# bigpon/QPNet

Hardware: AMD Instinct MI355X
Metric: train steps/sec (batch-1 chunk-steps of RF+20000 samples, aggregate over GPUs) (higher is better)
Workload: dtype f32; 1 GPU; config[1]: paper-size SI-QPNet (C=64,S=256,4F+4A) training step, forward+CE+backward+Adam on one chunk of 20900 samples (RF 946 + batch_length 19954), batch 1 per GPU; global_batch=1, parallelism=dp1 (utterance-sharded chunks, one flat-gradient all-reduce per step), backend=none, world_size=1, aux_1x1=frame rate (hoisted: K = 128 + one 4-deep step)

## Files before the change

qpnet_amd/csrc/train_bwd.hip:

```cpp
#include "train_common.h"
#include "train_post.h"
#include "qpn_handle.h"
#include <string.h>
#include <stdlib.h>
#include <math.h>

template <int MT>
__global__ __launch_bounds__(512) void k_post_bwd(TrainParams p, TrainBwd bw) {
    constexpr int TM = 16 * MT;
    extern __shared__ float sm[];
    const int S = p.S, Q = p.Q, LC = p.LC;
    const int ldp = tr_lda(Q > S ? Q : S), ldr = tr_lda(S);
    float* P = sm; float* R = sm + TM * ldp;
    const int b = blockIdx.y, t0 = blockIdx.x * TM;
    const int tid = threadIdx.x, lane = tid & 63, wave = tid >> 6;
    const int NTS = S / 16;
    const int npairs = (NTS + 1) / 2;
    const int np0 = wave < npairs ? wave : 0;
    const int pnt[2] = {2 * np0, (2 * np0 + 1 < NTS) ? 2 * np0 + 1 : 2 * np0};
    float my[2][MT][4], ms[2][MT][4];
    auto mask_load = [&](const float* src, float (&m)[2][MT][4]) {
#pragma unroll
        for (int j = 0; j < 2; ++j)
#pragma unroll
// ... 414 lines not shown
        }
        if constexpr (HOIST) {
            if (lane < 16) {
                float* dp = bw.DPA + cpoff + 16 * wave + lane;
                atomicAdd(dp, dacc[0]); atomicAdd(dp + C, dacc[1]); atomicAdd(dp + 2 * C, dacc[2]); atomicAdd(dp + 3 * C, dacc[3]);
                float* ep = bw.EB + (size_t)(l * TR_EB_SLOTS + (blockIdx.x & (TR_EB_SLOTS - 1))) * 2 * C + 16 * wave + lane;
                atomicAdd(ep, eacc[0]); atomicAdd(ep + C, eacc[1]);
            }
            if (tid < 16 && n0 + tid < N1) GWl[n0 + tid] = (Gp[tid] + Gp[16 + tid]) + (Gp[32 + tid] + Gp[48 + tid]);
        }
        store_rows(t + 1 < t_last ? t + 1 : t_last, sm + ((ti + 1) & 1) * 4 * 16 * ldx);
#pragma unroll
        for (int i = 0; i < 4; ++i) tprow[i] = tpnext[i];
        if constexpr (HOIST) {
#pragma unroll
            for (int i = 0; i < 4; ++i) { cwj[i] = nwj[i]; cpa[i] = npa[i]; }
            cpoff = npoff;
        }
    }
}

struct Wg2 {
    const float* A; const float* A2; size_t A_lstride; int lda, M;
    int rowsA;
    int bmode; const float* B1; const float* B2; size_t B_lstride; int ldb, N, Nvalid;
    int rowsB;
    const float* hup; const int* tap; int C, Ap;
    const int* xc;
    int nb, nlayers;
    float* slab; int gstage;
    int row0A[TR_MAXL], row0B[TR_MAXL], R[TR_MAXL];
    int goff[TR_MAXL], gbias[TR_MAXL], tap_off[TR_MAXL], dil[TR_MAXL];
    int ldc, ncol_groups;
};

struct Wg2L {
    const float* A; const float* A2; const float* B1; const float* B2; const float* hup; const int* tap;
    int lda, ldb, M, Ng, Nvalid, rowsA, rowsB, row0A, row0B, C, Ap, dil, nb, ncol0, rend;
    unsigned uR;
};

template <int NB>
__device__ __forceinline__ void wg_taps(const Wg2L& q, int rs, int (&tp)[NB], bool b_act, int b_row0, int b_rstep) {
#pragma unroll
    for (int k = 0; k < NB; ++k) {
        const int r = b_row0 + k * b_rstep, rr = rs + r;
        int v = 0;
        if (b_act && r < 32 && rr < q.rend) {
            const unsigned b = q.nb > 1 ? (unsigned)rr / q.uR : 0u; const int i = rr - (int)(b * q.uR);
            const int nloc = q.row0B + i;
            v = q.tap ? q.tap[(size_t)b * q.rowsB + nloc] : nloc - q.dil;
        }
        tp[k] = v;
    }
}

template <int BMODE, int NA, int NB>
__device__ __forceinline__ void wg_fetch(const Wg2L& q, int rs, float4 (&ra)[NA], float4 (&ra2)[NA], float4 (&rb)[NB], float4 (&rb2)[NB], const int (&tpv)[NB],
                                         bool a_act, int a_row0, int a_rstep, int a_col, bool b_act, int b_row0, int b_rstep, int b_col) {
#pragma unroll
    for (int k = 0; k < NA; ++k) {
        const int r = a_row0 + k * a_rstep, rr = rs + r;
        float4 v = make_float4(0.f, 0.f, 0.f, 0.f), v2 = v;
        if (a_act && r < 32 && rr < q.rend && a_col < q.M) {
            const unsigned b = q.nb > 1 ? (unsigned)rr / q.uR : 0u; const int i = rr - (int)(b * q.uR);
            const size_t o = ((size_t)b * q.rowsA + q.row0A + i) * q.lda + a_col;
// ... 155 lines not shown
    __shared__ float hcol[64];
    __shared__ float red[4];
    const int U = p.U, Ap = p.Ap, A = p.A;
    const int64_t q0 = (int64_t)p.F * U - p.N1;
    const int f = (int)(q0 / U) + fx;
    float dsum = 0.f;
    for (int a0 = 0; a0 < A; a0 += 64) {
        __syncthreads();
        if (tid < 64) hcol[tid] = (a0 + tid < A && f < p.F) ? p.h[((size_t)b * A + a0 + tid) * p.F + f] : 0.f;
        __syncthreads();
        for (int j = tid; j < U; j += nthr) {
            const int64_t n = (int64_t)f * U + j - q0;
            if (n < 0 || n >= p.N1 || f >= p.F) continue;
            const float* row = p.DHUP + ((size_t)b * p.N1 + n) * Ap + a0;
            float acc = 0.f;
            const int na = A - a0 < 64 ? A - a0 : 64;
            const int nq = na >> 2;
            float4 v[16];
#pragma unroll
            for (int q = 0; q < 16; ++q) v[q] = *(const float4*)(row + 4 * (q < nq ? q : 0));
#pragma unroll
            for (int q = 0; q < 16; ++q)
                if (q < nq) { acc += v[q].x * hcol[4 * q] + v[q].y * hcol[4 * q + 1] + v[q].z * hcol[4 * q + 2] + v[q].w * hcol[4 * q + 3]; dsum += (v[q].x + v[q].y) + (v[q].z + v[q].w); }
            for (int a = 4 * nq; a < na; ++a) { const float v1 = row[a]; acc += v1 * hcol[a]; dsum += v1; }
            atomicAdd(&p.gflat[p.up_w + j], acc * p.gscale);
        }
    }
    for (int s = 32; s >= 1; s >>= 1) dsum += __shfl_xor(dsum, s);
    if ((tid & 63) == 0) red[tid >> 6] = dsum;
    __syncthreads();
    if (tid == 0) { float a = 0.f; for (int k = 0; k < nthr / 64; ++k) a += red[k]; atomicAdd(&p.gflat[p.up_b], a * p.gscale); }
}

template <int BMODE, int MPW, int NT, bool TWO_A>
__device__ __forceinline__ void wgrad3_body(const Wg2& w, const int nch, const int ch, const int y, const int zg) {
    extern __shared__ float sm[];
    constexpr int RS = 32, Mp = 64 * MPW, Np = 16 * NT;
    constexpr int ldA = ((Mp + 15) / 32) * 32 + 16, ldB = ((Np + 15) / 32) * 32 + 16;
    constexpr int A4 = Mp / 4, ARS = 256 / A4, NA = RS / ARS;
    constexpr int B4 = Np / 4, BRS = 256 / B4, NB = (RS + BRS - 1) / BRS;
    static_assert(256 % A4 == 0 && RS % ARS == 0, "A staging must tile the stage's rows exactly");
    constexpr int BUF = RS * (ldA + ldB);
    float* As = sm; float* Bs = sm + RS * ldA;
    const int tid = threadIdx.x, lane = tid & 63, wave = tid >> 6;
    const int Rl = w.R[y];
    const int64_t total = (int64_t)Rl * w.nb;
    const int64_t per = ((total + nch - 1) / nch + RS - 1) / RS * RS;
    const int rbeg = (int)(per * ch), rend = (int)(per * ch + per < total ? per * ch + per : total);
    const float* A = w.A + (size_t)y * w.A_lstride;
    const float* A2 = TWO_A ? w.A2 + (size_t)y * w.A_lstride : nullptr;
    const float* B1 = BMODE == 4 ? nullptr : w.B1 + (size_t)y * w.B_lstride;
    const float* B2 = w.B2 ? w.B2 + (size_t)y * w.B_lstride : nullptr;
    const int* tap = BMODE == 3 ? w.tap + w.tap_off[y] : nullptr;
    const int row0A = w.row0A[y], row0B = w.row0B[y], ncol0 = zg * Np;
    const unsigned uR = (unsigned)(Rl > 0 ? Rl : 1);
    const bool multi = w.nb > 1;
    const int gbias = zg == 0 ? w.gbias[y] : -1, goff = w.goff[y];
    const int a_col = (tid % A4) * 4, a_row0 = tid / A4;
    const int b_col = (tid % B4) * 4, b_row0 = tid / B4;
    const int n = ncol0 + b_col;
    const bool b_act = tid < BRS * B4;
    const bool b_pad = n >= w.Nvalid;
    const float* bbase; int bstride; bool use_tap = false;
    if (BMODE == 3) {
        if (n < w.C) { bbase = B1 + n; bstride = w.C; }
        else if (n < 2 * w.C) { bbase = B1 + (n - w.C); bstride = w.C; use_tap = true; }
        else { bbase = w.hup + (b_pad ? 0 : n - 2 * w.C); bstride = w.Ap; }
    } else if (BMODE == 4) { bbase = nullptr; bstride = 0; }
    else { bbase = B1 + n; bstride = w.ldb; }
    const ptrdiff_t b2off = (BMODE == 2) ? (B2 - B1) : 0;

    f32x4 acc[MPW][NT];
#pragma unroll
    for (int a = 0; a < MPW; ++a)
#pragma unroll
        for (int b = 0; b < NT; ++b) acc[a][b] = (f32x4){0, 0, 0, 0};
    float4 cs4 = make_float4(0.f, 0.f, 0.f, 0.f);
    float4 ra[NA], ra2[NA], rb[NB], rb2[NB];
    int tpv[NB];
    int rbi[NB];
    unsigned okA = 0, okB = 0;

    const unsigned a_voff = (unsigned)a_row0 * (unsigned)w.lda + (unsigned)a_col, a_kstep = (unsigned)ARS * (unsigned)w.lda;
    const unsigned b_voff = (unsigned)b_row0 * (unsigned)w.ldb + (unsigned)n, b_kstep = (unsigned)BRS * (unsigned)w.ldb;

    auto rowsplit = [&](int rr, int& b, int& i) { if (multi) { b = (int)((unsigned)rr / uR); i = rr - b * (int)uR; } else { b = 0; i = rr; } };
    auto stage_fast = [&](int rs, int& b0, int& i0) {
        rowsplit(rs, b0, i0);
        return rs + RS <= rend && i0 + RS <= (int)uR;
    };
    auto taps = [&](int rs) {
        int b0, i0;
        if (stage_fast(rs, b0, i0)) {
            const int* tst = tap + ((size_t)b0 * w.rowsB + row0B + i0);
#pragma unroll
            for (int k = 0; k < NB; ++k) { const int r = b_row0 + k * BRS; tpv[k] = tst[r < RS ? r : b_row0]; }
            return;
        }
#pragma unroll
        for (int k = 0; k < NB; ++k) {
            const int r = b_row0 + k * BRS;
            int rr = rs + r; rr = rr < rend ? rr : rend - 1;
            int b, i; rowsplit(rr, b, i);
            const int nloc = row0B + i;
            tpv[k] = tap[(size_t)b * w.rowsB + nloc];
        }
    };
    auto fetch = [&](int rs) {
        const float* pa[NA]; const float* pb[NB]; const int* pi[NB];
        int b0, i0;
        if (stage_fast(rs, b0, i0)) {
            const float* Ast = A + ((size_t)b0 * w.rowsA + row0A + i0) * w.lda;
#pragma unroll
            for (int k = 0; k < NA; ++k) pa[k] = Ast + (k * a_kstep + a_voff);
            okA = ~0u;
            const size_t brow = (size_t)b0 * w.rowsB + row0B + i0;
            const float* bsrc = BMODE == 3 ? bbase + (size_t)b0 * w.rowsB * bstride : B1 + brow * w.ldb;
#pragma unroll
            for (int k = 0; k < NB; ++k) {
                const int r = b_row0 + k * BRS;
                if (BMODE == 4) pi[k] = w.xc + brow + (r < RS ? r : b_row0);
                else if (BMODE == 3) {
                    const unsigned row = use_tap ? (unsigned)tpv[k] : (unsigned)(row0B + i0 + (r < RS ? r : b_row0));
                    pb[k] = bsrc + __umul24(row, (unsigned)bstride);
                } else pb[k] = bsrc + ((r < RS ? k * b_kstep : 0u) + b_voff);
            }
            okB = b_pad ? 0u : ~0u;
        } else {
            okA = 0; okB = 0;
#pragma unroll
            for (int k = 0; k < NA; ++k) {
                const int r = a_row0 + k * ARS;
                int rr = rs + r; const bool ok = rr < rend; rr = ok ? rr : rend - 1;
                int b, i; rowsplit(rr, b, i);
                pa[k] = A + (((size_t)b * w.rowsA + row0A + i) * w.lda + a_col);
                okA |= ok ? 1u << k : 0u;
            }
#pragma unroll
            for (int k = 0; k < NB; ++k) {
                const int r = b_row0 + k * BRS;
                int rr = rs + r; const bool ok = r < RS && rr < rend && !b_pad; rr = rr < rend ? rr : rend - 1;
                int b, i; rowsplit(rr, b, i);
                const size_t row = (size_t)b * w.rowsB + ((BMODE == 3 && use_tap) ? tpv[k] : row0B + i);
                if (BMODE == 4) pi[k] = w.xc + row; else pb[k] = bbase + row * bstride;
                okB |= ok ? 1u << k : 0u;
            }
        }
#pragma unroll
        for (int k = 0; k < NA; ++k) {
            ra[k] = *(const float4*)pa[k];
            if (TWO_A) ra2[k] = *(const float4*)(pa[k] + (A2 - A));
        }
        if (b_act) {
#pragma unroll
            for (int k = 0; k < NB; ++k) {
                if (BMODE == 4) rbi[k] = *pi[k];
                else {
                    rb[k] = *(const float4*)pb[k];
                    if (BMODE == 2) rb2[k] = *(const float4*)(pb[k] + b2off);
                }
            }
        }
    };
    if (rbeg < rend) {
        if (BMODE == 3) taps(rbeg);
        fetch(rbeg);
        if (BMODE == 3 && rbeg + RS < rend) taps(rbeg + RS);
    }
    const int g = lane >> 4, cl = lane & 15;
    auto to_lds = [&](int buf) {
        float* Ab = As + buf * BUF; float* Bb = Bs + buf * BUF;
#pragma unroll
        for (int k = 0; k < NA; ++k) {
            float4 v = ra[k];
            if (TWO_A) { v.x += ra2[k].x; v.y += ra2[k].y; v.z += ra2[k].z; v.w += ra2[k].w; }
            { const bool ok = (okA >> k) & 1u; v.x = ok ? v.x : 0.f; v.y = ok ? v.y : 0.f; v.z = ok ? v.z : 0.f; v.w = ok ? v.w : 0.f; }
            cs4.x += v.x; cs4.y += v.y; cs4.z += v.z; cs4.w += v.w;
            *(float4*)(Ab + (size_t)(a_row0 + k * ARS) * ldA + a_col) = v;
        }
        if (b_act) {
#pragma unroll
            for (int k = 0; k < NB; ++k) {
                const int r = b_row0 + k * BRS;
                if (r < RS) {
                    float4 v;
                    if (BMODE == 4) { const int dlt = rbi[k] - n; v = make_float4(dlt == 0 ? 1.f : 0.f, dlt == 1 ? 1.f : 0.f, dlt == 2 ? 1.f : 0.f, dlt == 3 ? 1.f : 0.f); }
                    else v = rb[k];
                    if (BMODE == 1) { v.x = fmaxf(v.x, 0.f); v.y = fmaxf(v.y, 0.f); v.z = fmaxf(v.z, 0.f); v.w = fmaxf(v.w, 0.f); }
                    else if (BMODE == 2) { v.x *= rb2[k].x; v.y *= rb2[k].y; v.z *= rb2[k].z; v.w *= rb2[k].w; }
                    { const bool ok = (okB >> k) & 1u; v.x = ok ? v.x : 0.f; v.y = ok ? v.y : 0.f; v.z = ok ? v.z : 0.f; v.w = ok ? v.w : 0.f; }
                    *(float4*)(Bb + (size_t)r * ldB + b_col) = v;
                }
            }
        }
    };
    auto ksteps = [&](int buf, int k0, int k1) {
        const float* Ab = As + buf * BUF; const float* Bb = Bs + buf * BUF;
#pragma unroll
        for (int ks = k0; ks < k1; ++ks) {
            float bfr[NT];
#pragma unroll
            for (int nt = 0; nt < NT; ++nt) bfr[nt] = Bb[(4 * ks + g) * ldB + 16 * nt + cl];
#pragma unroll
            for (int mi = 0; mi < MPW; ++mi) {
                const float a = Ab[(4 * ks + g) * ldA + 16 * (wave + 4 * mi) + cl];
#pragma unroll
                for (int nt = 0; nt < NT; ++nt) acc[mi][nt] = __builtin_amdgcn_mfma_f32_16x16x4f32(a, bfr[nt], acc[mi][nt], 0, 0, 0);
            }
        }
    };
    for (int rs = rbeg; rs < rend; rs += RS) {
        to_lds(0);
        __syncthreads();
        if (rs + RS < rend) {
            fetch(rs + RS);
            if (BMODE == 3 && rs + 2 * RS < rend) taps(rs + 2 * RS);
        }
        ksteps(0, 0, RS / 4);
        __syncthreads();
    }
    float* out = w.slab + (size_t)ch * w.gstage;
#pragma unroll
    for (int mi = 0; mi < MPW; ++mi) {
        const int mt = wave + 4 * mi;
#pragma unroll
        for (int nt = 0; nt < NT; ++nt) {
#pragma unroll
            for (int i = 0; i < 4; ++i) {
                const int m = 16 * mt + 4 * (lane >> 4) + i, nn = 16 * nt + (lane & 15);
                out[goff + (size_t)m * w.ldc + ncol0 + nn] = acc[mi][nt][i];
            }
        }
    }
    if (gbias >= 0) {
        *(float4*)(sm + (size_t)a_row0 * Mp + a_col) = cs4;
        __syncthreads();
        if (tid < Mp) { float s = 0.f; for (int r = 0; r < ARS; ++r) s += sm[r * Mp + tid]; out[gbias + tid] = s; }
    }
}
template <int BMODE, int MPW, int NT, bool TWO_A, int MINW = 1>
__global__ __launch_bounds__(256, MINW) void k_wgrad3(Wg2 w, int nch) {
    wgrad3_body<BMODE, MPW, NT, TWO_A>(w, nch, blockIdx.x, blockIdx.y, blockIdx.z);
}

#ifndef QPN_WGRAD_MINW
#define QPN_WGRAD_MINW 2
#endif
template <int BMODE, int MPW, int NT, bool TWO_A>
static void launch_wgrad3_k(const Wg2& w, int nch, size_t lds, hipStream_t stream) {
    constexpr int MINW = (MPW == 4 && NT == 4 && !TWO_A) ? QPN_WGRAD_MINW : 1;
    if (lds > 64 * 1024) (void)hipFuncSetAttribute((const void*)k_wgrad3<BMODE, MPW, NT, TWO_A, MINW>, hipFuncAttributeMaxDynamicSharedMemorySize, (int)lds);
    hipLaunchKernelGGL((k_wgrad3<BMODE, MPW, NT, TWO_A, MINW>), dim3(nch, w.nlayers, w.ncol_groups), dim3(256), lds, stream, w, nch);
}
template <int BMODE, int MPW, int NT>
static bool wgrad3_fits(const Wg2& w) {
    const int Ng = w.N / w.ncol_groups;
    if (w.bmode != BMODE) return false;
    if (w.rowsB >= (1 << 24) || (int64_t)w.rowsB * (w.C > w.ldb ? w.C : w.ldb) >= (1ll << 32)) return false;
    if (w.M != 64 * MPW || Ng != 16 * NT || w.N % w.ncol_groups || (w.Nvalid != w.N && (w.ncol_groups != 1 || w.Nvalid % 4))) return false;
    if (BMODE == 3 && (w.ldb != w.C || w.ncol_groups != 1 || (w.C % 4) || (w.Ap % 4) || !w.tap)) return false;
    if (BMODE == 3) for (int l = 0; l < w.nlayers; ++l) if (w.tap_off[l] < 0) return false;
    return true;
}
template <int MPW, int NT> static constexpr size_t wgrad3_lds() { return (size_t)32 * (tr_ldt(64 * MPW) + tr_ldt(16 * NT)) * sizeof(float); }
template <int BMODE, int MPW, int NT>
static bool launch_wgrad3(const Wg2& w, int nch, hipStream_t stream) {
    if (!wgrad3_fits<BMODE, MPW, NT>(w)) return false;
    const size_t lds = wgrad3_lds<MPW, NT>();
    if (w.A2) launch_wgrad3_k<BMODE, MPW, NT, true>(w, nch, lds, stream);
    else launch_wgrad3_k<BMODE, MPW, NT, false>(w, nch, lds, stream);
    return true;
}
static bool wgrad3_any(const Wg2& w, int nch, bool generic, hipStream_t stream) {
    if (w.bmode == 4) return launch_wgrad3<4, 1, 8>(w, nch, stream) || launch_wgrad3<4, 1, 4>(w, nch, stream);
    if (generic) return false;
    switch (w.bmode) {
    case 3: return launch_wgrad3<3, 2, 11>(w, nch, stream) || launch_wgrad3<3, 2, 8>(w, nch, stream) || launch_wgrad3<3, 1, 7>(w, nch, stream);
    case 0: return launch_wgrad3<0, 1, 4>(w, nch, stream) || launch_wgrad3<0, 4, 4>(w, nch, stream);
    case 1: return launch_wgrad3<1, 4, 4>(w, nch, stream);
    default: return false;
    }
}

static int wgrad_col_groups(int M, int N) {
    const int nt_max = M <= 64 ? 4 : M <= 128 ? 12 : 8;
    for (int g = 1; g <= N / 16; ++g)
        if (N % g == 0 && (N / g) % 4 == 0 && (N / g + 15) / 16 <= nt_max) return g;
    return 1;
}

static bool wgrad2_any(const Wg2& w, int nch, bool generic, hipStream_t stream) {
    if (w.M > 256 && w.bmode != 4) {
        bool ok = true;
        for (int m0 = 0; m0 < w.M && ok; m0 += 256) {
            Wg2 sub = w;
            sub.A = w.A + m0; if (w.A2) sub.A2 = w.A2 + m0;
            sub.M = w.M - m0 < 256 ? w.M - m0 : 256;
            for (int l = 0; l < w.nlayers; ++l) { sub.goff[l] = w.goff[l] + m0 * w.ldc; if (w.gbias[l] >= 0) sub.gbias[l] = w.gbias[l] + m0; }
            sub.ncol_groups = wgrad_col_groups(sub.M, sub.N);
            ok = wgrad2_any(sub, nch, generic, stream);
        }
        return ok;
    }
    if (wgrad3_any(w, nch, generic, stream)) return true;
    switch (w.bmode) {
    case 4: return false;
    case 1: return wgrad2_mode<1>(w, nch, stream);
    case 2: return wgrad2_mode<2>(w, nch, stream);
    case 3: return wgrad2_mode<3>(w, nch, stream);
    default: return wgrad2_mode<0>(w, nch, stream);
    }
}

__global__ void k_reduce_grad_s(const float* __restrict__ slab, const int* __restrict__ gdst, const int* __restrict__ gdst_list, const int* __restrict__ gzero, int n_gzero,
                                int nch, int gstage, int64_t n, float* __restrict__ g, float scale, int append_scale, int s0, int s1, int skip0, int skip1, int tail,
                                const int* __restrict__ status, int flag_again) {
    int64_t i = (int64_t)blockIdx.x * blockDim.x + threadIdx.x + s0;
    if (flag_again && append_scale && i == s0) g[n + 1] = (status && *status) ? 1.f : 0.f;
    if (i < s1) {
        if (i >= skip0 && i < skip1) return;
        const int k0 = gdst[i], k1 = gdst[i + 1];
        if (k0 == k1) return;
        float a = 0.f;
        const float* sp = slab + i;
        int c = 0;
        for (; c + 8 <= nch; c += 8) {
            float v[8];
#pragma unroll
            for (int k = 0; k < 8; ++k) v[k] = sp[(size_t)(c + k) * gstage];
            a += ((v[0] + v[1]) + (v[2] + v[3])) + ((v[4] + v[5]) + (v[6] + v[7]));
        }
        for (; c < nch; ++c) a += sp[(size_t)c * gstage];
        a *= scale;
        for (int k = k0; k < k1; ++k) g[gdst_list[k]] = a;
        return;
    }
    if (!tail) return;
// ... 279 lines not shown
    hipLaunchKernelGGL((k_post_fb_w<MTW>), dim3((p.BL + 16 * MTW - 1) / (16 * MTW), p.B), dim3(512), ldsw, stream, p, bw, 1);
}

int qpn_launch_bwd(const TrainParams& p, const TrainBwd& bw, const TrainKnobs& k, const AuxGeom& ag, const StackQ* sq, hipStream_t stream, bool post_done) {
    const int C = p.C, S = p.S, Q = p.Q, L = p.L, B = p.B, N1 = p.N1, BL = p.BL;
    const TrainSlabs& sl = *bw.sl;
    const bool off32 = N1 < (1 << 24) && (int64_t)N1 * (p.LC > 2 * C ? p.LC : 2 * C) < (1ll << 32);
    const bool persist = C == 64 && (p.Ktp == 176 || p.hoist) && p.Ap <= 64 && off32 && k.persist_bwd;
    const bool stack_q = persist && k.stack_q_bwd && sq && sq->flags && p.qctl && qpn_stack_bwd_fits(p);
    const bool wr_summed = stack_q;
    const size_t nDX = (size_t)B * N1 * C;
    const size_t lds_post = (size_t)16 * (tr_lda(Q > S ? Q : S) + tr_lda(S)) * sizeof(float);
    const size_t lds_layer = (size_t)16 * (4 * tr_lda(C) + tr_lda(2 * C)) * sizeof(float);
    if (lds_post > 160 * 1024 || lds_layer > 160 * 1024) { qpn_set_error("backward tiles do not fit LDS"); return QPN_EINVAL; }
    hipStream_t side = bw.side; hipEvent_t ev_fork = bw.ev_fork, ev_join = bw.ev_join;
    const bool overlap = side && !qpn_prof_serial() && !k.serial;
    const bool post_wide = S == 256 && Q == 256 && C == 64 && (p.LC == 256 || p.LC == 512) && k.post_wide;
    const bool zero_in_post = post_wide && k.zero_in_post;
    if (post_done) { }
    else if (!zero_in_post) qpn_launch_zero_dx(p, bw, stream);
    if (post_done) { }
    else if (post_wide) {
        constexpr int MTW = 5;
        const size_t ldsw = (size_t)16 * MTW * tr_lda(256) * sizeof(float);
        QPN_HIP(hipFuncSetAttribute((const void*)k_post_bwd_w<MTW>, hipFuncAttributeMaxDynamicSharedMemorySize, (int)ldsw));
        hipLaunchKernelGGL((k_post_bwd_w<MTW>), dim3((BL + 16 * MTW - 1) / (16 * MTW), B), dim3(512), ldsw, stream, p, bw, zero_in_post ? 1 : 0);
    } else {
        if (lds_post > 48 * 1024) (void)hipFuncSetAttribute((const void*)k_post_bwd<1>, hipFuncAttributeMaxDynamicSharedMemorySize, (int)lds_post);
        hipLaunchKernelGGL((k_post_bwd<1>), dim3((BL + 15) / 16, B), dim3(512), lds_post, stream, p, bw);
    }
    qpn_prof_mark(PG_POST_BWD, stream);
    const int nch = bw.nch;
    int nch_side_ = nch;
    const bool gen = k.wgrad_generic;
    Wg2 wbase; memset(&wbase, 0, sizeof(wbase));
    wbase.slab = bw.slab; wbase.gstage = bw.gstage; wbase.nb = B; wbase.C = C; wbase.Ap = p.Ap; wbase.hup = p.HUP; wbase.tap = p.TAP; wbase.ncol_groups = 1;
    bool ok = true;
    auto launch_skip_post = [&](hipStream_t st) {
        Wg2 w = wbase;
        {
            w.nlayers = L;
            w.A = bw.DS0; w.A2 = nullptr; w.A_lstride = 0; w.lda = S; w.M = S; w.rowsA = BL;
            w.bmode = 0; w.B1 = p.TH; w.B2 = nullptr; w.B_lstride = nDX; w.ldb = C; w.N = C; w.Nvalid = C; w.rowsB = N1; w.ldc = C;
            w.ncol_groups = wgrad_col_groups(w.M, w.N);
            for (int l = 0; l < L; ++l) { w.row0A[l] = 0; w.row0B[l] = N1 - BL; w.R[l] = BL; w.goff[l] = sl.g_ws[l]; w.gbias[l] = l == 0 ? sl.g_bs : -1; w.tap_off[l] = -1; }
            ok = ok && wgrad2_any(w, nch_side_, gen, st);
            qpn_prof_mark(PG_WGRAD_SKIP, st);
        }
        {
            w.nlayers = 1; w.A_lstride = w.B_lstride = 0; w.B2 = nullptr; w.bmode = 1; w.rowsA = w.rowsB = BL;
            w.row0A[0] = w.row0B[0] = 0; w.R[0] = BL; w.tap_off[0] = -1;
            w.ncol_groups = S % 64 == 0 ? S / 64 : 1;
            w.A = bw.dlogits; w.lda = Q; w.M = Q; w.B1 = p.Y0; w.ldb = S; w.N = S; w.Nvalid = S; w.ldc = S; w.goff[0] = sl.g_p2; w.gbias[0] = sl.g_bp2;
            if (Q == S && k.post_pair) {
                w.nlayers = 2;
                w.A_lstride = (size_t)(bw.DY0 - bw.dlogits); w.B_lstride = (size_t)(p.S0 - p.Y0);
                w.row0A[1] = w.row0B[1] = 0; w.R[1] = BL; w.tap_off[1] = -1; w.goff[1] = sl.g_p1; w.gbias[1] = sl.g_bp1;
                ok = ok && wgrad2_any(w, nch_side_, gen, st);
            } else {
                ok = ok && wgrad2_any(w, nch_side_, gen, st);
                w.A = bw.DY0; w.lda = S; w.M = S; w.B1 = p.S0; w.goff[0] = sl.g_p1; w.gbias[0] = sl.g_bp1;
                ok = ok && wgrad2_any(w, nch_side_, gen, st);
            }
            qpn_prof_mark(PG_WGRAD_POST, st);
        }
    };
    auto build_w1 = [&]() {
        Wg2 w = wbase;
// ... 117 lines not shown
```

qpnet_amd/csrc/train_common.h:

```cpp
#pragma once
#include "qpn_common.h"

typedef float f32x4 __attribute__((ext_vector_type(4)));

#define TR_MAXL QPN_MAX_LAYERS

__host__ __device__ static inline int tr_lda(int K) { return ((K + 29) / 32) * 32 + 2; }
__host__ __device__ static inline int tr_ldt(int N) { return ((N + 15) / 32) * 32 + 16; }

struct TrLayer {
    int adaptive, dilation;
    int s_in, s_out;
    int tap_off;
    int w1_f4, wr_f4;
    int w1t_f4, wrt_f4;
    int bias1, biasr;
};

struct TrainParams {
    int C, S, Q, A, Ap, L, U;
    int B, T, F, Td, BL, N1, N0, maxd;
    int Kt, Ktp;
    int LC;
    const float* flat;
// ... 48 lines not shown
    float* slab;
    const int* gdst; const int* gdst_list;
    const int* gzero; int n_gzero;
    int nch, gstage;
    int64_t n_params;
    const struct TrainSlabs* sl;
    float gscale;
    int append_scale;
    const int* status;
    hipStream_t side; hipEvent_t ev_fork, ev_join, ev_mid;
    hipEvent_t ev_early; int* early_recorded;
};


struct AuxGeom { int auxS[TR_MAXL], auxT[TR_MAXL], bias1[TR_MAXL], s_out[TR_MAXL]; };
struct AuxArgs {
    const float* flat; const float* h; float* PA; float* bp; const float* DPA; const float* EB; const float* GW; float* gflat;
    float gscale; int C, A, L, B, F, U, N1, nfr, ffirst; int64_t up_w, up_b;
    AuxGeom g;
};
static inline AuxArgs tr_aux_args(const TrainParams& p, const TrainBwd* bw, const AuxGeom& ag) {
    AuxArgs a; a.flat = p.flat; a.h = p.h; a.PA = p.PA; a.bp = p.bp; a.DPA = bw ? bw->DPA : nullptr; a.EB = bw ? bw->EB : nullptr; a.GW = bw ? bw->GW : nullptr;
    a.gflat = bw ? bw->gflat : nullptr; a.gscale = bw ? bw->gscale : 1.f;
    a.C = p.C; a.A = p.A; a.L = p.L; a.B = p.B; a.F = p.F; a.U = p.U; a.N1 = p.N1; a.nfr = p.nfr; a.ffirst = p.ffirst; a.up_w = p.up_w; a.up_b = p.up_b; a.g = ag;
    return a;
}
struct TrainKnobs {
    bool serial;
    bool stack_q_fwd, stack_q_bwd;
    int stack_wgs, stack_wgs_bwd;
    bool persist_fwd, persist_bwd;
    bool wgrad_generic;
    int wgrad_chunks, wgrad_chunks_side;
    bool post_fuse;
    bool up_side, reduce_early, wr_side;
    bool post_pair, zero_in_post, post_wide;
    bool xcd_swizzle;
    bool ce_separate;
    bool event_fence;
    bool aux_hoist;
    bool test_stack_gives_up;
};
void qpn_train_knobs_parse(TrainKnobs& k);

#define TR_QHEAD_STRIDE 1056
#define TR_QHDR_WORDS 17920
struct StackQ {
    unsigned* flags;
    unsigned* head;
    unsigned* stats;
    unsigned* abort;
    const int4* tab;
    unsigned epoch;
    unsigned epoch_pub;
    unsigned spin_limit;
    int total, nq;
};

__host__ __device__ __forceinline__ int tr_pa_off(const TrainParams& p, int l, int b, int n0) {
    const int q = p.F * p.U - p.N1 + n0;
    return ((l * p.B + b) * (p.nfr + 1) + (q / p.U - p.ffirst)) * 2 * p.C;
}

__device__ __forceinline__ void tr_queue_entry_fwd(const TrainParams& p, int pos, int4& a, int4& b) {
    const bool valid = pos < p.qtotal;
    const int ps = valid ? pos : 0;
// ... 259 lines not shown
```

qpnet_amd/csrc/train_host.hip:

```cpp
#include "train_common.h"
#include "qpn_handle.h"
#include <algorithm>
#include <string.h>

int qpn_launch_fwd(const TrainParams& p, const TrainKnobs& k, const AuxGeom& ag, const StackQ* sq, hipStream_t stream, const TrainBwd* fuse_post_bwd);
void qpn_stack_fill(TrainParams& p);
int qpn_launch_ce(const float* logits, const int64_t* tgt, int64_t tgt_stride, int B, int BL, int Q, float* dlogits, double* loss, int* status, bool loss_cleared, hipStream_t stream);
int qpn_launch_bwd(const TrainParams& p, const TrainBwd& bw, const TrainKnobs& k, const AuxGeom& ag, const StackQ* sq, hipStream_t stream, bool post_done);
int qpn_launch_fwd_gemm(const TrainParams& p, const TrainGemm& w, hipStream_t stream);
int qpn_launch_bwd_gemm(const TrainParams& p, const TrainBwd& bw, const TrainGemm& w, hipStream_t stream);
int qpn_launch_adam(float* w, const float* g, float* m, float* v, int64_t n, int step, float lr, float b1, float b2, float eps, float wd, const float* den, int* status,
                    int* h_status, double* h_loss, const double* d_loss, hipStream_t stream);
int qpn_launch_adam_clip(float* w, const float* g, float* m, float* v, int64_t n, int step, float lr, float b1, float b2, float eps, float wd, const float* den, int* status,
                         int* h_status, double* h_loss, const double* d_loss, float max_norm, double* part, double* d_norm, double* h_norm, hipStream_t stream);

#define LOSS_SLOT 72

struct TrainState {
    std::vector<int> h_wmap;
    std::vector<int> h_bstart, h_blist;
    std::vector<int> h_gsrc;
    int* d_wmap; float* d_wp; int* d_bstart; int* d_blist; float* d_bp; int n_bias;
    int* d_gdst; int* d_gdst_list; int* d_gzero; int n_gzero;
    bool hoist;
// ... 10 lines not shown
    double* h_loss_pinned; hipEvent_t ev_loss[2]; bool loss_pending[2]; int loss_newest;
    double* d_gnorm; bool gnorm_last;
    bool gnorm_slot[2];
    double gnorm_collected; bool gnorm_collected_valid;
    bool fwd_valid;
    bool loss_clear;
    bool use_gemm;
    int* d_ctmap; float* d_ct;
    std::vector<int> h_gmap; int* d_gmap; float* d_gwp;
    TrainGemm gm;
    int64_t generation;
    hipStream_t side; hipEvent_t ev_fork, ev_join, ev_mid;
    hipEvent_t ev_early; int early_recorded; int64_t early_first;
    int64_t bwd_generation;
    const float* post_bwd_dlogits;
    bool post_bwd_done;
    bool stack_disabled;
    unsigned* d_sq; size_t sq_pos_cap, sq_per_dir;
    StackQ sqf, sqb;
};

static int env_int(const char* name, int dflt) { const char* e = getenv(name); return (e && *e) ? atoi(e) : dflt; }
void qpn_train_knobs_parse(TrainKnobs& k) {
    k.serial = env_int("QPN_TRAIN_SERIAL", 0) != 0;
    k.stack_q_fwd = env_int("QPN_STACK_QUEUE", 1) != 0;
    k.stack_q_bwd = k.stack_q_fwd && env_int("QPN_STACK_QUEUE_BWD", 1) != 0;
    k.stack_wgs = env_int("QPN_STACK_WGS", 0); if (k.stack_wgs < 0 || k.stack_wgs > 4096) k.stack_wgs = 0;
    k.stack_wgs_bwd = env_int("QPN_STACK_WGS_BWD", 0); if (k.stack_wgs_bwd < 0 || k.stack_wgs_bwd > 4096) k.stack_wgs_bwd = 0;
    k.persist_fwd = env_int("QPN_LAYER_PERSIST", 1) != 0;
    k.persist_bwd = env_int("QPN_LAYER_BWD_PERSIST", 1) != 0;
    k.wgrad_generic = getenv("QPN_WGRAD_GENERIC") != nullptr;
    k.wgrad_chunks = env_int("QPN_WGRAD_CHUNKS", 0); if (k.wgrad_chunks < 1 || k.wgrad_chunks > 512) k.wgrad_chunks = 0;
    k.wgrad_chunks_side = env_int("QPN_WGRAD_CHUNKS_SIDE", 0); if (k.wgrad_chunks_side < 1 || k.wgrad_chunks_side > 512) k.wgrad_chunks_side = 0;
    k.up_side = env_int("QPN_UP_SIDE", 1) != 0;
    k.reduce_early = env_int("QPN_REDUCE_EARLY", 1) != 0;
    k.wr_side = env_int("QPN_WR_SIDE", 1) != 0;
    k.post_fuse = env_int("QPN_POST_FUSE", 1) != 0;
    k.post_pair = env_int("QPN_POST_WGRAD_PAIR", 1) != 0;
    k.zero_in_post = env_int("QPN_ZERO_IN_POST", 1) != 0;
    k.post_wide = env_int("QPN_POST_WIDE", 1) != 0;
    k.xcd_swizzle = getenv("QPN_NO_XCD_SWIZZLE") == nullptr;
    k.ce_separate = getenv("QPN_CE_SEPARATE") != nullptr;
    k.event_fence = env_int("QPN_EVENT_FENCE", 0) == 1;
    k.aux_hoist = env_int("QPN_AUX_HOIST", 1) != 0;
    k.test_stack_gives_up = false;
#ifdef QPN_TESTING
    k.test_stack_gives_up = env_int("QPN_TEST_STACK_GIVES_UP", 0) == 1;
#endif
}

int qpn_num_cus() {
    static int cached[64] = {0};
    int dev = 0;
    if (hipGetDevice(&dev) != hipSuccess || dev < 0 || dev >= 64) return 256;
    if (!cached[dev]) { int n = 0; if (hipDeviceGetAttribute(&n, hipDeviceAttributeMultiprocessorCount, dev) != hipSuccess || n < 1) n = 256; cached[dev] = n; }
    return cached[dev];
}

struct Prof { bool on = false; bool overlapped = false; std::vector<hipEvent_t> ev; std::vector<int> grp; std::vector<hipStream_t> st; size_t used = 0; };
static thread_local Prof g_prof;
bool qpn_prof_active() { return g_prof.on; }
bool qpn_prof_serial() { return g_prof.on && !g_prof.overlapped; }
void qpn_prof_mark(int group, hipStream_t stream) {
    Prof& P = g_prof;
    if (!P.on) return;
    if (P.used == P.ev.size()) { hipEvent_t e; if (hipEventCreate(&e) != hipSuccess) return; P.ev.push_back(e); P.grp.push_back(0); P.st.push_back(nullptr); }
// ... 755 lines not shown
```

Baseline: 1472 steps/s.

## Stage wgrad A operand directly in registers with triple-buffered prefetch

Adds a register-direct path for the weight-gradient MFMA kernel on selected shapes. The A operand is loaded from global memory straight into MFMA-ready register vectors two stages ahead, and only B goes through double-buffered LDS, so each stage needs one barrier instead of two. The aim is to cut LDS traffic and synchronisation and to overlap loads with MFMA work. In exchange it raises register pressure, and launch bounds ask for two waves per SIMD. It is on by default behind an env knob, and optional timestamp instrumentation is compiled in only under a debug macro.

After: 1420 steps/s. -3.6%, worse.

```diff
diff --git a/qpnet_amd/csrc/train_bwd.hip b/qpnet_amd/csrc/train_bwd.hip
--- a/qpnet_amd/csrc/train_bwd.hip
+++ b/qpnet_amd/csrc/train_bwd.hip
@@ -470,6 +470,9 @@
     int row0A[TR_MAXL], row0B[TR_MAXL], R[TR_MAXL];
     int goff[TR_MAXL], gbias[TR_MAXL], tap_off[TR_MAXL], dil[TR_MAXL];
     int ldc, ncol_groups;
+#ifdef QPN_WGRAD_STAMPS
+    unsigned* stamps;
+#endif
 };
 
 struct Wg2L {
@@ -691,7 +694,15 @@
     if (tid == 0) { float a = 0.f; for (int k = 0; k < nthr / 64; ++k) a += red[k]; atomicAdd(&p.gflat[p.up_b], a * p.gscale); }
 }
 
-template <int BMODE, int MPW, int NT, bool TWO_A>
+#ifdef QPN_WGRAD_STAMPS
+#define WG_STAMP(i) do { __builtin_amdgcn_sched_barrier(0); if (wg_st) { unsigned long long t_; asm volatile("s_memtime %0\n\ts_waitcnt lgkmcnt(0)" : "=s"(t_) :: "memory"); \
+    if (tid == 0 && wg_stage < 16) wg_st[8 * wg_stage + (i)] = (unsigned)t_; } __builtin_amdgcn_sched_barrier(0); } while (0)
+#define WG_STAMP_NEXT() (++wg_stage)
+#else
+#define WG_STAMP(i) do { } while (0)
+#define WG_STAMP_NEXT() do { } while (0)
+#endif
+template <int BMODE, int MPW, int NT, bool TWO_A, bool DIRECT_A>
 __device__ __forceinline__ void wgrad3_body(const Wg2& w, const int nch, const int ch, const int y, const int zg) {
     extern __shared__ float sm[];
     constexpr int RS = 32, Mp = 64 * MPW, Np = 16 * NT;
@@ -729,6 +740,11 @@
     else { bbase = B1 + n; bstride = w.ldb; }
     const ptrdiff_t b2off = (BMODE == 2) ? (B2 - B1) : 0;
 
+#ifdef QPN_WGRAD_STAMPS
+    constexpr int wg_slot = (BMODE == 3 && MPW == 2 && NT == 8) ? 0 : (BMODE == 0 && MPW == 4) ? 1 : (BMODE == 1 && MPW == 4) ? 2 : -1;
+    unsigned* const wg_st = (wg_slot >= 0 && !TWO_A && w.stamps && ch == 5 && zg == 0 && y == (BMODE == 1 ? 0 : 3)) ? w.stamps + 600 + 128 * wg_slot : nullptr;
+    int wg_stage = 0;
+#endif
     f32x4 acc[MPW][NT];
 #pragma unroll
     for (int a = 0; a < MPW; ++a)
@@ -748,12 +764,12 @@
         rowsplit(rs, b0, i0);
         return rs + RS <= rend && i0 + RS <= (int)uR;
     };
-    auto taps = [&](int rs) {
+    auto taps_to = [&](int (&tp)[NB], int rs) __attribute__((always_inline)) {
         int b0, i0;
         if (stage_fast(rs, b0, i0)) {
             const int* tst = tap + ((size_t)b0 * w.rowsB + row0B + i0);
 #pragma unroll
-            for (int k = 0; k < NB; ++k) { const int r = b_row0 + k * BRS; tpv[k] = tst[r < RS ? r : b_row0]; }
+            for (int k = 0; k < NB; ++k) { const int r = b_row0 + k * BRS; tp[k] = tst[r < RS ? r : b_row0]; }
             return;
         }
 #pragma unroll
@@ -762,9 +778,10 @@
             int rr = rs + r; rr = rr < rend ? rr : rend - 1;
             int b, i; rowsplit(rr, b, i);
             const int nloc = row0B + i;
-            tpv[k] = tap[(size_t)b * w.rowsB + nloc];
+            tp[k] = tap[(size_t)b * w.rowsB + nloc];
         }
     };
+    auto taps = [&](int rs) { taps_to(tpv, rs); };
     auto fetch = [&](int rs) {
         const float* pa[NA]; const float* pb[NB]; const int* pi[NB];
         int b0, i0;
@@ -821,6 +838,155 @@
             }
         }
     };
+    if constexpr (DIRECT_A) {
+        static_assert(!TWO_A && (BMODE == 0 || BMODE == 1 || BMODE == 3) && (MPW == 2 || MPW == 4), "register-direct staging: one A array, 8- or 16-byte words");
+        static_assert(BRS * B4 == 256 && NB * BRS == RS, "B staging must tile the stage's rows exactly with every thread active");
+        typedef float AV __attribute__((ext_vector_type(MPW)));
+#define GLOBAL_AS __attribute__((address_space(1)))
+        constexpr int KS = RS / 4;
+        struct Set { AV a[KS]; unsigned ok; };
+        Set S0, S1, S2;
+        const int g = lane >> 4, cl = lane & 15;
+        const int ad_col = (Mp / 4) * wave + MPW * cl;
+        const unsigned ad_voff = (unsigned)g * (unsigned)w.lda + (unsigned)ad_col, ad_kstep = 4u * (unsigned)w.lda;
+        auto fetch_a = [&](Set& s, int rs) __attribute__((always_inline)) {
+            const float* pa[KS];
+            int b0, i0;
+            if (stage_fast(rs, b0, i0)) {
+                const float* Ast = A + ((size_t)b0 * w.rowsA + row0A + i0) * w.lda;
+#pragma unroll
+                for (int k = 0; k < KS; ++k) pa[k] = Ast + (k * ad_kstep + ad_voff);
+                s.ok = ~0u;
+            } else {
+                s.ok = 0;
+#pragma unroll
+                for (int k = 0; k < KS; ++k) {
+                    int rr = rs + 4 * k + g; const bool ok = rr < rend; rr = ok ? rr : rend - 1;
+                    int b, i; rowsplit(rr, b, i);
+                    pa[k] = A + (((size_t)b * w.rowsA + row0A + i) * w.lda + ad_col);
+                    s.ok |= ok ? 1u << k : 0u;
+                }
+            }
+#pragma unroll
+            for (int k = 0; k < KS; ++k) s.a[k] = *(const GLOBAL_AS AV*)pa[k];
+        };
+        auto fetch_b = [&](int rs) __attribute__((always_inline)) {
+            const float* pb[NB];
+            int b0, i0;
+            if (stage_fast(rs, b0, i0)) {
+                const size_t brow = (size_t)b0 * w.rowsB + row0B + i0;
+                const float* bsrc = BMODE == 3 ? bbase + (size_t)b0 * w.rowsB * bstride : B1 + brow * w.ldb;
+#pragma unroll
+                for (int k = 0; k < NB; ++k) {
+                    if (BMODE == 3) {
+                        const unsigned row = use_tap ? (unsigned)tpv[k] : (unsigned)(row0B + i0 + b_row0 + k * BRS);
+                        pb[k] = bsrc + __umul24(row, (unsigned)bstride);
+                    } else pb[k] = bsrc + (k * b_kstep + b_voff);
+                }
+                okB = b_pad ? 0u : ~0u;
+            } else {
+                okB = 0;
+#pragma unroll
+                for (int k = 0; k < NB; ++k) {
+                    int rr = rs + b_row0 + k * BRS; const bool ok = rr < rend && !b_pad; rr = rr < rend ? rr : rend - 1;
+                    int b, i; rowsplit(rr, b, i);
+                    const size_t row = (size_t)b * w.rowsB + ((BMODE == 3 && use_tap) ? tpv[k] : row0B + i);
+                    pb[k] = bbase + row * bstride;
+                    okB |= ok ? 1u << k : 0u;
+                }
+            }
+#pragma unroll
+            for (int k = 0; k < NB; ++k) { const f32x4 v = *(const GLOBAL_AS f32x4*)pb[k]; rb[k] = make_float4(v[0], v[1], v[2], v[3]); }
+        };
+        auto b_to_lds = [&](float* Bb) __attribute__((always_inline)) {
+#pragma unroll
+            for (int k = 0; k < NB; ++k) {
+                float4 v = rb[k];
+                if (BMODE == 1) { v.x = fmaxf(v.x, 0.f); v.y = fmaxf(v.y, 0.f); v.z = fmaxf(v.z, 0.f); v.w = fmaxf(v.w, 0.f); }
+                { const bool ok = (okB >> k) & 1u; v.x = ok ? v.x : 0.f; v.y = ok ? v.y : 0.f; v.z = ok ? v.z : 0.f; v.w = ok ? v.w : 0.f; }
+                *(float4*)(Bb + (size_t)(b_row0 + k * BRS) * ldB + b_col) = v;
+            }
+        };
+        float cs[MPW];
+#pragma unroll
+        for (int j = 0; j < MPW; ++j) cs[j] = 0.f;
+        constexpr int YOUNGER = 2 * KS + NB + (BMODE == 3 ? NB : 0);
+        auto stage = [&](Set& cur, Set& nn, int rs, const float* Bcur, float* Bnxt) __attribute__((always_inline)) {
+            WG_STAMP(0);
+            const int rs2 = rs + 2 * RS < rend ? rs + 2 * RS : rs;
+            fetch_a(nn, rs2);
+            WG_STAMP(1);
+            __builtin_amdgcn_s_waitcnt(0x0F70 | (YOUNGER & 15) | ((YOUNGER >> 4) << 14));
+            WG_STAMP(2);
+#pragma unroll
+            for (int ks = 0; ks < KS; ++ks) {
+                float bfr[NT];
+#pragma unroll
+                for (int nt = 0; nt < NT; ++nt) bfr[nt] = Bcur[(4 * ks + g) * ldB + 16 * nt + cl];
+#pragma unroll
+                for (int j = 0; j < MPW; ++j)
+#pragma unroll
+                    for (int nt = 0; nt < NT; ++nt) acc[j][nt] = __builtin_amdgcn_mfma_f32_16x16x4f32(cur.a[ks][j], bfr[nt], acc[j][nt], 0, 0, 0);
+            }
+            WG_STAMP(3);
+            if (gbias >= 0) {
+#pragma unroll
+                for (int ks = 0; ks < KS; ++ks) {
+                    const bool ok = (cur.ok >> ks) & 1u;
+#pragma unroll
+                    for (int j = 0; j < MPW; ++j) cs[j] += ok ? cur.a[ks][j] : 0.f;
+                }
+            }
+            b_to_lds(Bnxt);
+            fetch_b(rs2);
+            if (BMODE == 3) taps(rs + 3 * RS < rend ? rs + 3 * RS : rs);
+            WG_STAMP(4);
+            __syncthreads();
+            WG_STAMP(5);
+            WG_STAMP_NEXT();
+        };
+        if (rbeg < rend) {
+            float* const Bs0 = sm; float* const Bs1 = sm + RS * ldB;
+            const int rs1 = rbeg + RS < rend ? rbeg + RS : rbeg;
+            if (BMODE == 3) taps(rbeg);
+            fetch_a(S0, rbeg);
+            fetch_b(rbeg);
+            if (BMODE == 3) taps(rs1);
+            fetch_a(S1, rs1);
+            b_to_lds(Bs0);
+            fetch_b(rs1);
+            if (BMODE == 3) taps(rbeg + 2 * RS < rend ? rbeg + 2 * RS : rbeg);
+            __syncthreads();
+            for (int rs = rbeg;;) {
+                stage(S0, S2, rs, Bs0, Bs1); rs += RS; if (rs >= rend) break;
+                stage(S1, S0, rs, Bs1, Bs0); rs += RS; if (rs >= rend) break;
+                stage(S2, S1, rs, Bs0, Bs1); rs += RS; if (rs >= rend) break;
+                stage(S0, S2, rs, Bs1, Bs0); rs += RS; if (rs >= rend) break;
+                stage(S1, S0, rs, Bs0, Bs1); rs += RS; if (rs >= rend) break;
+                stage(S2, S1, rs, Bs1, Bs0); rs += RS; if (rs >= rend) break;
+            }
+        }
+        float* out = w.slab + (size_t)ch * w.gstage;
+#pragma unroll
+        for (int j = 0; j < MPW; ++j)
+#pragma unroll
+            for (int nt = 0; nt < NT; ++nt)
+#pragma unroll
+                for (int i = 0; i < 4; ++i) {
+                    const int m = (Mp / 4) * wave + MPW * (4 * g + i) + j, nn = 16 * nt + cl;
+                    out[goff + (size_t)m * w.ldc + ncol0 + nn] = acc[j][nt][i];
+                }
+        if (gbias >= 0) {
+#pragma unroll
+            for (int j = 0; j < MPW; ++j) {
+                float v = cs[j];
+                v += __shfl_xor(v, 16); v += __shfl_xor(v, 32);
+                if (g == 0) out[gbias + ad_col + j] = v;
+            }
+        }
+#undef GLOBAL_AS
+        return;
+    }
     if (rbeg < rend) {
         if (BMODE == 3) taps(rbeg);
         fetch(rbeg);
@@ -869,14 +1035,21 @@
         }
     };
     for (int rs = rbeg; rs < rend; rs += RS) {
+        WG_STAMP(0);
         to_lds(0);
+        WG_STAMP(1);
         __syncthreads();
+        WG_STAMP(2);
         if (rs + RS < rend) {
             fetch(rs + RS);
             if (BMODE == 3 && rs + 2 * RS < rend) taps(rs + 2 * RS);
         }
+        WG_STAMP(3);
         ksteps(0, 0, RS / 4);
+        WG_STAMP(4);
         __syncthreads();
+        WG_STAMP(5);
+        WG_STAMP_NEXT();
     }
     float* out = w.slab + (size_t)ch * w.gstage;
 #pragma unroll
@@ -897,19 +1070,34 @@
         if (tid < Mp) { float s = 0.f; for (int r = 0; r < ARS; ++r) s += sm[r * Mp + tid]; out[gbias + tid] = s; }
     }
 }
+template <int BMODE, int MPW, int NT, bool TWO_A>
+constexpr bool wgrad3_direct() { return !TWO_A && ((MPW == 4 && NT == 4 && (BMODE == 0 || BMODE == 1)) || (BMODE == 3 && MPW == 2 && NT == 8)); }
 template <int BMODE, int MPW, int NT, bool TWO_A, int MINW = 1>
-__global__ __launch_bounds__(256, MINW) void k_wgrad3(Wg2 w, int nch) {
-    wgrad3_body<BMODE, MPW, NT, TWO_A>(w, nch, blockIdx.x, blockIdx.y, blockIdx.z);
+__global__ __launch_bounds__(256, (wgrad3_direct<BMODE, MPW, NT, TWO_A>() && MINW < 2) ? 2 : MINW) void k_wgrad3(Wg2 w, int nch) {
+    wgrad3_body<BMODE, MPW, NT, TWO_A, wgrad3_direct<BMODE, MPW, NT, TWO_A>()>(w, nch, blockIdx.x, blockIdx.y, blockIdx.z);
+}
+template <int BMODE, int MPW, int NT, bool TWO_A, int MINW = 1>
+__global__ __launch_bounds__(256, MINW) void k_wgrad3_lds(Wg2 w, int nch) {
+    wgrad3_body<BMODE, MPW, NT, TWO_A, false>(w, nch, blockIdx.x, blockIdx.y, blockIdx.z);
 }
 
 #ifndef QPN_WGRAD_MINW
 #define QPN_WGRAD_MINW 2
 #endif
+template <int MPW, int NT> static size_t wgrad3_lds() { return (size_t)32 * (tr_ldt(64 * MPW) + tr_ldt(16 * NT)) * sizeof(float); }
+template <int NT> static size_t wgrad3_lds_direct() { return (size_t)2 * 32 * tr_ldt(16 * NT) * sizeof(float); }
 template <int BMODE, int MPW, int NT, bool TWO_A>
-static void launch_wgrad3_k(const Wg2& w, int nch, size_t lds, hipStream_t stream) {
+static void launch_wgrad3_k(const Wg2& w, int nch, bool direct, hipStream_t stream) {
     constexpr int MINW = (MPW == 4 && NT == 4 && !TWO_A) ? QPN_WGRAD_MINW : 1;
-    if (lds > 64 * 1024) (void)hipFuncSetAttribute((const void*)k_wgrad3<BMODE, MPW, NT, TWO_A, MINW>, hipFuncAttributeMaxDynamicSharedMemorySize, (int)lds);
-    hipLaunchKernelGGL((k_wgrad3<BMODE, MPW, NT, TWO_A, MINW>), dim3(nch, w.nlayers, w.ncol_groups), dim3(256), lds, stream, w, nch);
+    const dim3 grid(nch, w.nlayers, w.ncol_groups);
+    const size_t lds = wgrad3_lds<MPW, NT>();
+    if constexpr (wgrad3_direct<BMODE, MPW, NT, TWO_A>()) {
+        if (direct) hipLaunchKernelGGL((k_wgrad3<BMODE, MPW, NT, TWO_A, MINW>), grid, dim3(256), wgrad3_lds_direct<NT>(), stream, w, nch);
+        else hipLaunchKernelGGL((k_wgrad3_lds<BMODE, MPW, NT, TWO_A, MINW>), grid, dim3(256), lds, stream, w, nch);
+    } else {
+        if (lds > 64 * 1024) (void)hipFuncSetAttribute((const void*)k_wgrad3<BMODE, MPW, NT, TWO_A, MINW>, hipFuncAttributeMaxDynamicSharedMemorySize, (int)lds);
+        hipLaunchKernelGGL((k_wgrad3<BMODE, MPW, NT, TWO_A, MINW>), grid, dim3(256), lds, stream, w, nch);
+    }
 }
 template <int BMODE, int MPW, int NT>
 static bool wgrad3_fits(const Wg2& w) {
@@ -921,22 +1109,22 @@
     if (BMODE == 3) for (int l = 0; l < w.nlayers; ++l) if (w.tap_off[l] < 0) return false;
     return true;
 }
-template <int MPW, int NT> static constexpr size_t wgrad3_lds() { return (size_t)32 * (tr_ldt(64 * MPW) + tr_ldt(16 * NT)) * sizeof(float); }
 template <int BMODE, int MPW, int NT>
-static bool launch_wgrad3(const Wg2& w, int nch, hipStream_t stream) {
+static bool launch_wgrad3(const Wg2& w, int nch, bool direct, hipStream_t stream) {
     if (!wgrad3_fits<BMODE, MPW, NT>(w)) return false;
-    const size_t lds = wgrad3_lds<MPW, NT>();
-    if (w.A2) launch_wgrad3_k<BMODE, MPW, NT, true>(w, nch, lds, stream);
-    else launch_wgrad3_k<BMODE, MPW, NT, false>(w, nch, lds, stream);
+    if (w.A2) launch_wgrad3_k<BMODE, MPW, NT, true>(w, nch, direct, stream);
+    else launch_wgrad3_k<BMODE, MPW, NT, false>(w, nch, direct, stream);
     return true;
 }
-static bool wgrad3_any(const Wg2& w, int nch, bool generic, hipStream_t stream) {
-    if (w.bmode == 4) return launch_wgrad3<4, 1, 8>(w, nch, stream) || launch_wgrad3<4, 1, 4>(w, nch, stream);
-    if (generic) return false;
+struct WgSel { bool generic, direct; };
+static bool wgrad3_any(const Wg2& w, int nch, WgSel sel, hipStream_t stream) {
+    const bool d = sel.direct;
+    if (w.bmode == 4) return launch_wgrad3<4, 1, 8>(w, nch, d, stream) || launch_wgrad3<4, 1, 4>(w, nch, d, stream);
+    if (sel.generic) return false;
     switch (w.bmode) {
-    case 3: return launch_wgrad3<3, 2, 11>(w, nch, stream) || launch_wgrad3<3, 2, 8>(w, nch, stream) || launch_wgrad3<3, 1, 7>(w, nch, stream);
-    case 0: return launch_wgrad3<0, 1, 4>(w, nch, stream) || launch_wgrad3<0, 4, 4>(w, nch, stream);
-    case 1: return launch_wgrad3<1, 4, 4>(w, nch, stream);
+    case 3: return launch_wgrad3<3, 2, 11>(w, nch, d, stream) || launch_wgrad3<3, 2, 8>(w, nch, d, stream) || launch_wgrad3<3, 1, 7>(w, nch, d, stream);
+    case 0: return launch_wgrad3<0, 1, 4>(w, nch, d, stream) || launch_wgrad3<0, 4, 4>(w, nch, d, stream);
+    case 1: return launch_wgrad3<1, 4, 4>(w, nch, d, stream);
     default: return false;
     }
 }
@@ -948,7 +1136,7 @@
     return 1;
 }
 
-static bool wgrad2_any(const Wg2& w, int nch, bool generic, hipStream_t stream) {
+static bool wgrad2_any(const Wg2& w, int nch, WgSel sel, hipStream_t stream) {
     if (w.M > 256 && w.bmode != 4) {
         bool ok = true;
         for (int m0 = 0; m0 < w.M && ok; m0 += 256) {
@@ -957,11 +1145,11 @@
             sub.M = w.M - m0 < 256 ? w.M - m0 : 256;
             for (int l = 0; l < w.nlayers; ++l) { sub.goff[l] = w.goff[l] + m0 * w.ldc; if (w.gbias[l] >= 0) sub.gbias[l] = w.gbias[l] + m0; }
             sub.ncol_groups = wgrad_col_groups(sub.M, sub.N);
-            ok = wgrad2_any(sub, nch, generic, stream);
+            ok = wgrad2_any(sub, nch, sel, stream);
         }
         return ok;
     }
-    if (wgrad3_any(w, nch, generic, stream)) return true;
+    if (wgrad3_any(w, nch, sel, stream)) return true;
     switch (w.bmode) {
     case 4: return false;
     case 1: return wgrad2_mode<1>(w, nch, stream);
@@ -1307,8 +1495,11 @@
     qpn_prof_mark(PG_POST_BWD, stream);
     const int nch = bw.nch;
     int nch_side_ = nch;
-    const bool gen = k.wgrad_generic;
+    const WgSel gen = {k.wgrad_generic, k.wgrad_direct};
     Wg2 wbase; memset(&wbase, 0, sizeof(wbase));
+#ifdef QPN_WGRAD_STAMPS
+    wbase.stamps = p.qctl;
+#endif
     wbase.slab = bw.slab; wbase.gstage = bw.gstage; wbase.nb = B; wbase.C = C; wbase.Ap = p.Ap; wbase.hup = p.HUP; wbase.tap = p.TAP; wbase.ncol_groups = 1;
     bool ok = true;
     auto launch_skip_post = [&](hipStream_t st) {
diff --git a/qpnet_amd/csrc/train_common.h b/qpnet_amd/csrc/train_common.h
--- a/qpnet_amd/csrc/train_common.h
+++ b/qpnet_amd/csrc/train_common.h
@@ -104,6 +104,7 @@
     bool persist_fwd, persist_bwd;
     bool wgrad_generic;
     int wgrad_chunks, wgrad_chunks_side;
+    bool wgrad_direct;
     bool post_fuse;
     bool up_side, reduce_early, wr_side;
     bool post_pair, zero_in_post, post_wide;
diff --git a/qpnet_amd/csrc/train_host.hip b/qpnet_amd/csrc/train_host.hip
--- a/qpnet_amd/csrc/train_host.hip
+++ b/qpnet_amd/csrc/train_host.hip
@@ -66,6 +66,7 @@
     k.wgrad_generic = getenv("QPN_WGRAD_GENERIC") != nullptr;
     k.wgrad_chunks = env_int("QPN_WGRAD_CHUNKS", 0); if (k.wgrad_chunks < 1 || k.wgrad_chunks > 512) k.wgrad_chunks = 0;
     k.wgrad_chunks_side = env_int("QPN_WGRAD_CHUNKS_SIDE", 0); if (k.wgrad_chunks_side < 1 || k.wgrad_chunks_side > 512) k.wgrad_chunks_side = 0;
+    k.wgrad_direct = env_int("QPN_WGRAD_DIRECT", 1) != 0;
     k.up_side = env_int("QPN_UP_SIDE", 1) != 0;
     k.reduce_early = env_int("QPN_REDUCE_EARLY", 1) != 0;
     k.wr_side = env_int("QPN_WR_SIDE", 1) != 0;
```
